# antekone/libarchive

Measured on AMD Instinct MI355X. Metric: decompressed MiB/s (whole node), lz4 filter, XXH32 verified, bit-exact, higher is better.
Workload: dtype u8; 1 GPU; C2: raw-format + lz4 filter, 16.00 GiB decoded per GPU, 262144 independent 64 KiB blocks per GPU in frames of 16, block+content+header XXH32 verified; compressed_bytes_per_gpu=7527480016, decoded_bytes_per_gpu=17179869184, unique_region_mib=1024, tiles=16, collectives=RCCL (nccl backend), expand_kernel=auto

## Files before the change

### include/la_gpu.h

```cpp
#ifndef LA_GPU_H
#define LA_GPU_H

#include <stddef.h>
#include <stdint.h>

#ifdef __cplusplus
extern "C" {
#endif

#define LA_GPU_ABI_VERSION 3

typedef enum la_rc {
	LA_OK            = 0,
	LA_ERR_NO_DEVICE = -1,
	LA_ERR_HIP       = -2,
	LA_ERR_ARG       = -3,
	LA_ERR_NOMEM     = -4
} la_rc;

typedef struct la_gpu_ctx la_gpu_ctx;

int         la_gpu_abi_version(void);
int         la_gpu_device_count(void);
int         la_gpu_open(int device, la_gpu_ctx **out);
// ... 116 lines not shown
	uint32_t flags;
	uint32_t content_sum;
	uint32_t reserved;
} la_lz4_frame;

typedef struct la_batch_summary {
	uint64_t total_out;
	uint32_t n_bad_units;
	uint32_t n_bad_frames;
	uint32_t first_bad_unit;
	uint32_t first_bad_frame;
	uint32_t first_zero_unit;
	uint32_t reserved;
} la_batch_summary;

#define LA_LZ4_OPT_GENERAL_ONLY 1u
#define LA_LZ4_OPT_NO_VERIFY    2u
#define LA_LZ4_OPT_PARSE_V1     4u

#define LA_LZ4_OPT_EXPAND_INORDER 8u

#define LA_LZ4_OPT_SEARCH_IN_EXPAND 16u

typedef struct la_lz4_batch {
	const uint8_t      *d_src;
	uint64_t            src_bytes;
	const la_lz4_block *d_blocks;
	uint32_t            n_blocks;
	const la_lz4_frame *d_frames;
	uint32_t            n_frames;
	uint8_t            *d_dst;
	uint64_t            dst_cap;
	uint32_t           *d_out_len;
	uint64_t           *d_dst_off;
	uint32_t           *d_block_status;
	uint32_t           *d_frame_status;
	la_batch_summary   *d_summary;
	uint32_t            options;
	uint32_t            hist_len;
	const void         *d_carry_in;
	void               *d_carry_out;
} la_lz4_batch;
#define LA_XXH_CARRY_BYTES 64u

uint64_t la_gpu_lz4_workspace_bytes(uint32_t n_blocks, uint64_t src_bytes);

// ... 453 lines not shown
```

### libarchive_amd/_native.py

```python
import ctypes as C
import os

import numpy as np

_PKG = os.path.dirname(os.path.abspath(__file__))
GPU_LIB_PATH = os.environ.get("LA_GPU_LIB") or os.path.join(_PKG, "csrc", "libla_gpu.so")
HOST_LIB_PATH = os.path.join(_PKG, "host", "libla_host.so")

LA_OK = 0

LZ4_BLOCK_DTYPE = np.dtype([("src_off", "<u8"), ("src_len", "<u4"), ("dst_cap", "<u4"),
                            ("flags", "<u4"), ("block_sum", "<u4")])
LZ4_FRAME_DTYPE = np.dtype([("desc_off", "<u8"), ("desc_len", "<u4"), ("first_block", "<u4"),
                            ("n_blocks", "<u4"), ("flags", "<u4"), ("content_sum", "<u4"),
                            ("reserved", "<u4")])
HASH_JOB_DTYPE = np.dtype([("off", "<u8"), ("len", "<u4"), ("seed", "<u4")])
SUMMARY_DTYPE = np.dtype([("total_out", "<u8"), ("n_bad_units", "<u4"), ("n_bad_frames", "<u4"),
                          ("first_bad_unit", "<u4"), ("first_bad_frame", "<u4"),
                          ("first_zero_unit", "<u4"), ("reserved", "<u4")])
GZ_MEMBER_DTYPE = np.dtype([("src_off", "<u8"), ("src_len", "<u4"), ("dst_cap", "<u4"), ("dst_off", "<u8")])
GZ_RESULT_DTYPE = np.dtype([("status", "<u4"), ("out_len", "<u4"), ("consumed", "<u4"), ("crc32", "<u4")])
assert LZ4_BLOCK_DTYPE.itemsize == 24 and LZ4_FRAME_DTYPE.itemsize == 32
assert HASH_JOB_DTYPE.itemsize == 16 and SUMMARY_DTYPE.itemsize == 32

LA_LZ4B_STORED, LA_LZ4B_CHECKSUM, LA_LZ4B_DEPENDENT, LA_LZ4B_FIRST = 1, 2, 4, 8
LA_LZ4F_CONTENT_SUM, LA_LZ4F_HEADER_SUM, LA_LZ4F_CONT, LA_LZ4F_OPEN, LA_LZ4F_HASHED = 1, 2, 4, 8, 16
LA_LZ4_OPT_GENERAL_ONLY, LA_LZ4_OPT_NO_VERIFY, LA_LZ4_OPT_PARSE_V1, LA_LZ4_OPT_EXPAND_INORDER = 1, 2, 4, 8
LA_LZ4_OPT_SEARCH_IN_EXPAND = 16
LA_GPU_ABI_VERSION = 3
LA_ST_OK, LA_ST_GZ_DATA, LA_ST_GZ_TRUNCATED, LA_ST_GZ_OUT_FULL, LA_ST_GZ_NO_TRAILER = 0, 5, 6, 9, 10
LA_ST_GZ_PIECE_END, LA_ST_GZ_NEEDS_HISTORY = 18, 19
(LA_GZ_OPT_NO_VERIFY, LA_GZ_OPT_WAVE_KERNEL, LA_GZ_OPT_LANE_KERNEL, LA_GZ_OPT_TWO_PHASE, LA_GZ_OPT_RAW,
 LA_GZ_OPT_EXPAND_INORDER, LA_GZ_OPT_PIECES) = 1, 2, 4, 8, 16, 32, 64
LA_GZ_OPT_CHAIN = 128
LA_GZ_OPT_BLOCK_STARTS = 256
LA_GZ_OPT_START_BIT_SHIFT = 16

(LA_END_EOF, LA_END_TRUNCATED, LA_END_MALFORMED, LA_END_MALFORMED_SKIP, LA_END_EMPTY_FRAME,
 LA_END_NEED_MORE, LA_END_GZ_NO_TRAILER, LA_END_GZ_TOO_LARGE) = range(8)


class NativeLibraryMissing(RuntimeError):
    pass


class _Lz4BatchC(C.Structure):
    _fields_ = [
        ("d_src", C.c_void_p), ("src_bytes", C.c_uint64),
        ("d_blocks", C.c_void_p), ("n_blocks", C.c_uint32),
        ("d_frames", C.c_void_p), ("n_frames", C.c_uint32),
        ("d_dst", C.c_void_p), ("dst_cap", C.c_uint64),
# ... 558 lines not shown
```

### libarchive_amd/csrc/la_api.hip

```cpp
#include "la_dev.h"
#include <stdio.h>
#include <stdlib.h>
#include <string.h>
#include <new>

#define LA_MAX_SLICES 8
#define LA_GZ_LANES_MIN 8192u
#define LA_PROF_MAX_RANGES 64

struct la_gpu_ctx {
	int device;
	hipStream_t own_stream;
	hipStream_t stream;
	hipEvent_t ev0, ev1;
	hipEvent_t mark;
	void *ws;
	uint64_t ws_bytes;
	uint32_t *lz4_deps;
	uint64_t lz4_deps_cap;
	uint8_t *lz4_plan;
	hipStream_t aux_stream;
	hipEvent_t slice_ev[LA_MAX_SLICES + 1];
	int prof_on;
	int prof_n;
	hipEvent_t prof_a[LA_PROF_MAX_RANGES], prof_b[LA_PROF_MAX_RANGES];
	const char *prof_name[LA_PROF_MAX_RANGES];
	char err[256];
};

static void prof_begin(la_gpu_ctx *c) { c->prof_n = 0; }
static int prof_open(la_gpu_ctx *c, const char *name, hipStream_t s)
{
	if (!c->prof_on || c->prof_n >= LA_PROF_MAX_RANGES)
		return -1;
	int h = c->prof_n++;
	c->prof_name[h] = name;
	(void)hipEventRecord(c->prof_a[h], s);
	return h;
}
static void prof_close(la_gpu_ctx *c, int h, hipStream_t s)
{
	if (h >= 0)
		(void)hipEventRecord(c->prof_b[h], s);
}

// ... 34 lines not shown
	*out = NULL;
	int n = 0;
	if (hipGetDeviceCount(&n) != hipSuccess || n <= 0 || device < 0 || device >= n)
		return LA_ERR_NO_DEVICE;
	la_gpu_ctx *c = new (std::nothrow) la_gpu_ctx();
	if (!c)
		return LA_ERR_NOMEM;
	memset(c, 0, sizeof(*c));
	c->device = device;
	if (hipSetDevice(device) != hipSuccess ||
	    hipStreamCreateWithFlags(&c->own_stream, hipStreamNonBlocking) != hipSuccess ||
	    hipEventCreate(&c->ev0) != hipSuccess || hipEventCreate(&c->ev1) != hipSuccess ||
	    hipEventCreateWithFlags(&c->mark, hipEventDisableTiming) != hipSuccess) {
		delete c;
		return LA_ERR_NO_DEVICE;
	}
	for (int i = 0; i < LA_PROF_MAX_RANGES; i++) {
		(void)hipEventCreate(&c->prof_a[i]);
		(void)hipEventCreate(&c->prof_b[i]);
	}
	(void)hipStreamCreateWithFlags(&c->aux_stream, hipStreamNonBlocking);
	for (int i = 0; i <= LA_MAX_SLICES; i++)
		(void)hipEventCreateWithFlags(&c->slice_ev[i], hipEventDisableTiming);
	c->stream = c->own_stream;
	*out = c;
	return LA_OK;
}

void la_gpu_close(la_gpu_ctx *c)
{
	if (!c)
		return;
	(void)hipSetDevice(c->device);
	(void)hipStreamSynchronize(c->stream);
	if (c->ws) (void)hipFree(c->ws);
	if (c->lz4_deps) (void)hipFree(c->lz4_deps);
	if (c->lz4_plan) (void)hipFree(c->lz4_plan);
	(void)hipEventDestroy(c->ev0);
	(void)hipEventDestroy(c->ev1);
	(void)hipEventDestroy(c->mark);
	for (int i = 0; i < LA_PROF_MAX_RANGES; i++) {
		(void)hipEventDestroy(c->prof_a[i]);
		(void)hipEventDestroy(c->prof_b[i]);
	}
	for (int i = 0; i <= LA_MAX_SLICES; i++)
		(void)hipEventDestroy(c->slice_ev[i]);
	(void)hipStreamSynchronize(c->aux_stream);
	(void)hipStreamDestroy(c->aux_stream);
	(void)hipStreamDestroy(c->own_stream);
	delete c;
}

int la_gpu_set_stream(la_gpu_ctx *c, void *hip_stream)
{
	if (!c) return LA_ERR_ARG;
	c->stream = hip_stream ? (hipStream_t)hip_stream : c->own_stream;
	return LA_OK;
}

int la_gpu_sync(la_gpu_ctx *c)
{
	if (!c) return LA_ERR_ARG;
	HIPCHK(c, hipStreamSynchronize(c->stream));
	return LA_OK;
}

const char *la_gpu_last_error(const la_gpu_ctx *c) { return c ? c->err : "no context"; }

int la_gpu_reserve(la_gpu_ctx *c, uint64_t bytes)
// ... 179 lines not shown
{
	lz4_ws w;
	lz4_ws_carve(&w, NULL, n_blocks, src_bytes, true);
	return w.total;
}

static int lz4_deps_reserve(la_gpu_ctx *c, uint64_t words)
{
	if (words <= c->lz4_deps_cap)
		return LA_OK;
	HIPCHK(c, hipSetDevice(c->device));
	HIPCHK(c, hipStreamSynchronize(c->stream));
	HIPCHK(c, hipStreamSynchronize(c->aux_stream));
	c->lz4_deps_cap = 0;
	if (c->lz4_deps) { HIPCHK(c, hipFree(c->lz4_deps)); c->lz4_deps = NULL; }
	if (c->lz4_plan) { HIPCHK(c, hipFree(c->lz4_plan)); c->lz4_plan = NULL; }
	words = (words + 0x3FFFFull) & ~0x3FFFFull;
	HIPCHK(c, hipMalloc((void **)&c->lz4_deps, words * sizeof(uint32_t)));
	HIPCHK(c, hipMalloc((void **)&c->lz4_plan, words));
	c->lz4_deps_cap = words;
	return LA_OK;
}

static bool lz4_uses_deps(const la_lz4_batch *bt)
{
	return !(bt->options & (LA_LZ4_OPT_GENERAL_ONLY | LA_LZ4_OPT_SEARCH_IN_EXPAND)) && bt->n_blocks &&
	    ((bt->options & LA_LZ4_OPT_EXPAND_INORDER) == 0 || !la_lz4_expand_inorder_takes(bt->src_bytes));
}

int la_gpu_lz4_decode(la_gpu_ctx *c, const la_lz4_batch *bt)
{
	if (!c || !bt)
		return LA_ERR_ARG;
	if (!bt->d_dst_off || (bt->n_blocks && (!bt->d_src || !bt->d_blocks || !bt->d_dst || !bt->d_out_len ||
	    !bt->d_block_status)))
		return LA_ERR_ARG;
	if (bt->n_frames && (!bt->d_frames || !bt->d_frame_status))
		return LA_ERR_ARG;
	const bool fast = !(bt->options & LA_LZ4_OPT_GENERAL_ONLY);
	const bool verify = !(bt->options & LA_LZ4_OPT_NO_VERIFY);
	const bool poll = (bt->options & LA_LZ4_OPT_EXPAND_INORDER) == 0 || !la_lz4_expand_inorder_takes(bt->src_bytes);
	lz4_ws w;
	lz4_ws_carve(&w, NULL, bt->n_blocks, bt->src_bytes, fast);
	if (w.total > c->ws_bytes) {
		int rc = la_gpu_reserve(c, w.total);
		if (rc != LA_OK) return rc;
	}
	lz4_ws_carve(&w, (uint8_t *)c->ws, bt->n_blocks, bt->src_bytes, fast);
	const bool with_deps = lz4_uses_deps(bt);
	if (with_deps) {
		int rc = lz4_deps_reserve(c, w.table_cap);
		if (rc != LA_OK) return rc;
	}
	hipStream_t sx = c->stream;
	hipStream_t sp = c->aux_stream;
	const uint32_t n = bt->n_blocks;
	const la_expand_job xj = {	 bt->d_src, bt->src_bytes, bt->d_blocks, n, bt->d_dst, bt->dst_cap, bt->d_dst_off,
	    bt->d_out_len, bt->d_block_status, w.nseq, fast ? w.table : NULL, w.table_off,
	    LA_LZ4_LONG_SEQ_BYTES,
	    with_deps ? c->lz4_deps : NULL, with_deps ? c->lz4_plan : NULL };

	prof_begin(c);
	HIPCHK(c, hipEventRecord(c->slice_ev[LA_MAX_SLICES], sx));
	HIPCHK(c, hipStreamWaitEvent(sp, c->slice_ev[LA_MAX_SLICES], 0));

	if (n)
		HIPCHK(c, hipMemsetAsync(bt->d_block_status, 0, (size_t)n * sizeof(uint32_t), sp));
	if (fast) {
		la_launch_lz4_table_caps(sp, bt->d_blocks, n, w.caps);
		la_launch_scan_u32(sp, w.caps, n, w.table_off, w.scan);
	}
	if (verify && n)
		HIPCHK(c, hipMemsetAsync(w.sum_status, 0, (size_t)n * sizeof(uint32_t), sp));
	if (bt->options & LA_LZ4_OPT_PARSE_V1) {
		if (verify && n)
			prof_range(c, "lz4_block_sums", sp, [&] { la_launch_lz4_block_sums(sp, bt->d_src, bt->d_blocks, n, w.sum_status); });
		prof_range(c, "lz4_parse", sp, [&] {
			la_launch_lz4_parse(sp, bt->d_src, bt->src_bytes, bt->d_blocks, n, bt->d_out_len, w.nseq,
			    bt->d_block_status, fast ? w.table : NULL, w.table_off, w.table_cap);
		});
	} else {
		prof_range(c, "lz4_parse", sp, [&] {
			la_launch_lz4_parse_staged(sp, bt->d_src, bt->src_bytes, bt->d_blocks, n, bt->d_out_len, w.nseq,
			    bt->d_block_status, verify ? w.sum_status : NULL, fast ? w.table : NULL, w.table_off, w.table_cap);
		});
	}
	HIPCHK(c, hipEventRecord(c->slice_ev[0], sp));

	HIPCHK(c, hipStreamWaitEvent(sx, c->slice_ev[0], 0));
	prof_range(c, "scan", sx, [&] { la_launch_scan_u32(sx, bt->d_out_len, n, bt->d_dst_off, w.scan); });
	if (with_deps)
		prof_range(c, "lz4_deps", sx, [&] { la_launch_lz4_deps(sx, xj, c->lz4_deps, c->lz4_plan); });

	prof_range(c, fast ? "lz4_expand_general" : "lz4_expand", sx, [&] { la_launch_lz4_expand_general(sx, xj, bt->hist_len); });
	if (fast && poll)
		prof_range(c, "lz4_expand_big", sx, [&] { la_launch_lz4_expand_fast_big(sx, xj, w.big); });
	const uint32_t nsl = (fast && n >= 4u * 8192u) ? 4u : 1u;
	if (bt->n_frames && !verify)
		HIPCHK(c, hipMemsetAsync(bt->d_frame_status, 0, (size_t)bt->n_frames * sizeof(uint32_t), sx));
	for (uint32_t i = 0; i < nsl; i++) {
		const uint32_t first = (uint32_t)((uint64_t)n * i / nsl), last = (uint32_t)((uint64_t)n * (i + 1) / nsl);
		const la_expand_job sj = xj.slice(first, last - first);
		if (fast)
			prof_range(c, "lz4_expand", sx, [&] { (poll ? la_launch_lz4_expand_fast : la_launch_lz4_expand_inorder)(sx, sj); });
		if (bt->n_frames && verify) {
			HIPCHK(c, hipEventRecord(c->slice_ev[1 + i], sx));
			HIPCHK(c, hipStreamWaitEvent(sp, c->slice_ev[1 + i], 0));
			prof_range(c, "lz4_frame_sums", sp, [&] {
				la_launch_lz4_frame_sums(sp, bt->d_src, bt->d_dst, bt->d_frames, bt->n_frames,
				    bt->d_dst_off, bt->dst_cap, bt->d_frame_status, i ? first + 1 : 0u, last,
				    bt->d_carry_in, bt->d_carry_out,
				    i + 1 == nsl);
			});
		}
	}
	HIPCHK(c, hipEventRecord(c->slice_ev[LA_MAX_SLICES - 1], sp));
	HIPCHK(c, hipStreamWaitEvent(sx, c->slice_ev[LA_MAX_SLICES - 1], 0));
	if (verify)
		la_launch_lz4_merge_status(sx, w.sum_status, n, bt->d_block_status);
	if (bt->d_summary)
		prof_range(c, "summary", sx, [&] {
			la_launch_lz4_summary(sx, bt->d_out_len, bt->d_block_status, n, bt->d_frame_status, bt->n_frames, bt->d_dst_off, bt->d_summary);
		});
	HIPCHK(c, hipGetLastError());
// ... 671 lines not shown
```

### libarchive_amd/csrc/la_dev.h

```cpp
#ifndef LA_DEV_H
#define LA_DEV_H

#include <hip/hip_runtime.h>
#include <stdint.h>
#include "../../include/la_gpu.h"

#define LA_WAVE 64

__device__ __forceinline__ uint32_t ld_u32(const uint8_t *p)
{
	uint32_t v;
	__builtin_memcpy(&v, p, 4);
	return v;
}
__device__ __forceinline__ uint4 ld_u128(const uint8_t *p)
{
	uint4 v;
	__builtin_memcpy(&v, p, 16);
	return v;
}
__device__ __forceinline__ uint32_t rotl32(uint32_t x, int r)
{
	return __builtin_rotateleft32(x, r);
}

#define XXH_P1 0x9E3779B1u
#define XXH_P2 0x85EBCA77u
#define XXH_P3 0xC2B2AE3Du
// ... 332 lines not shown
	uint64_t off;
	template <typename T> T *take(uint64_t count, uint64_t align = alignof(T))
	{
		off = (off + align - 1) & ~(align - 1);
		T *p = base ? (T *)(void *)(base + off) : nullptr;
		off += count * sizeof(T);
		return p;
	}
};


void la_launch_xxh32_many(hipStream_t s, const uint8_t *d_base, const la_hash_job *d_jobs,
    uint32_t n, uint32_t *d_out);
void la_launch_crc32_many(hipStream_t s, const uint8_t *d_base, const la_hash_job *d_jobs,
    uint32_t n, uint32_t *d_out);
void la_launch_adler32_many(hipStream_t s, const uint8_t *d_base, const la_hash_job *d_jobs,
    uint32_t n, uint32_t *d_out);
void la_launch_lz4_block_sums(hipStream_t s, const uint8_t *d_src, const la_lz4_block *d_blocks,
    uint32_t n, uint32_t *d_status);
void la_launch_lz4_frame_sums(hipStream_t s, const uint8_t *d_src, const uint8_t *d_dst,
    const la_lz4_frame *d_frames, uint32_t n_frames, const uint64_t *d_dst_off,
    uint64_t dst_cap, uint32_t *d_frame_status, uint32_t end_lo, uint32_t end_hi,
    const void *d_carry_in, void *d_carry_out, int row );
void la_launch_lz4_merge_status(hipStream_t s, const uint32_t *d_sum_status, uint32_t n, uint32_t *d_status);

struct la_lz4_seq {
	uint16_t lit_src;
	uint16_t lit_len;
	uint16_t dst;
	uint16_t off;
};

#define LA_LZ4_FAST_MAXSEQ 4096u
#define LA_INFLATE_MAXSEQ 12288u

__host__ __device__ __forceinline__ bool la_lz4_fast_eligible(const la_lz4_block &b)
{
	return !(b.flags & (LA_LZ4B_STORED | LA_LZ4B_DEPENDENT)) && b.dst_cap <= 65536u && b.src_len <= 65536u;
}

#define LA_LZ4_LONG_SEQ_BYTES 512u
__host__ __device__ __forceinline__ bool la_lz4_long_sequences(uint32_t nseq, uint32_t out_len, uint32_t thr)
{
	return thr != 0 && nseq != 0xFFFFFFFFu && (uint64_t)nseq * thr <= out_len;
}

// ... 125 lines not shown
	uint32_t long_thr;
	const uint32_t *deps;
	const uint8_t *lit_plan;

	la_expand_job slice(uint32_t first, uint32_t count) const
	{
		return la_expand_job{ src, src_bytes, blocks + first, count, dst, dst_cap, dst_off + first, out_len + first,
		    status + first, nseq + first, table, table_off + first, long_thr, deps, lit_plan };
	}
};

void la_launch_lz4_table_caps(hipStream_t s, const la_lz4_block *d_blocks, uint32_t n, uint32_t *d_caps);
void la_launch_lz4_parse(hipStream_t s, const uint8_t *d_src, uint64_t src_bytes,
    const la_lz4_block *d_blocks, uint32_t n, uint32_t *d_out_len, uint32_t *d_nseq,
    uint32_t *d_status, la_lz4_seq *d_table , const uint64_t *d_table_off,
    uint64_t table_cap );
void la_launch_lz4_parse_staged(hipStream_t s, const uint8_t *d_src, uint64_t src_bytes,
    const la_lz4_block *d_blocks, uint32_t n, uint32_t *d_out_len, uint32_t *d_nseq,
    uint32_t *d_status, uint32_t *d_sum_status, la_lz4_seq *d_table, const uint64_t *d_table_off,
    uint64_t table_cap);
void la_launch_lz4_expand_general(hipStream_t s, const la_expand_job &j, uint32_t hist_len);
void la_launch_lz4_expand_fast(hipStream_t s, const la_expand_job &j);
void la_launch_lz4_expand_fast_big(hipStream_t s, const la_expand_job &j, uint32_t *d_big );
void la_launch_lz4_deps(hipStream_t s, const la_expand_job &j, uint32_t *d_deps, uint8_t *d_plan);

bool la_lz4_expand_inorder_takes(uint64_t src_bytes);
void la_launch_lz4_expand_inorder(hipStream_t s, const la_expand_job &j);

uint64_t la_zstd_workspace_bytes(uint32_t n_frames);
void la_launch_zstd_frames(hipStream_t s, const uint8_t *d_src, uint64_t src_bytes, const la_zstd_frame *d_frames, uint32_t n,
    uint8_t *d_dst, uint64_t dst_cap, la_zstd_result *d_results, uint8_t *ws, uint32_t options,
    const uint32_t *d_only );
uint64_t la_zstd_blocks_workspace_bytes(uint32_t n_frames, uint64_t src_bytes, uint64_t dst_cap);
const uint32_t *la_zstd_blocks_todo(const uint8_t *ws);
void la_launch_zstd_blocks(hipStream_t s, const uint8_t *d_src, uint64_t src_bytes, const la_zstd_frame *d_frames, uint32_t n,
    uint8_t *d_dst, uint64_t dst_cap, la_zstd_result *d_results, uint8_t *ws, uint32_t options);

uint64_t la_bzip2_workspace_bytes(uint32_t n, uint32_t level);
uint32_t la_bzip2_max_blocks(uint32_t level);
uint64_t la_bzip2_scan_ws_bytes(uint64_t src_bytes);
void la_launch_bzip2_scan(hipStream_t s, const uint8_t *d_src, uint64_t src_bytes, la_bz2_cand *d_cands, uint32_t cap,
    uint32_t *d_count, uint8_t *ws);
void la_launch_bzip2_measure(hipStream_t s, const la_bz2_batch *bt, uint8_t *ws);
void la_launch_bzip2_walk(hipStream_t s, const la_bz2_batch *bt, uint8_t *ws);
void la_launch_bzip2_emit(hipStream_t s, const la_bz2_batch *bt, uint8_t *ws);
void la_launch_bzip2_verify(hipStream_t s, const la_bz2_batch *bt, uint8_t *ws);
// ... 134 lines not shown
```

### libarchive_amd/csrc/la_hash.hip

```cpp
#include "la_dev.h"


__global__ __launch_bounds__(256) void xxh32_many_kernel(const uint8_t *__restrict__ base,
    const la_hash_job *__restrict__ jobs, uint32_t n, uint32_t *__restrict__ out)
{
	uint32_t i = blockIdx.x * blockDim.x + threadIdx.x;
	if (i >= n)
		return;
	la_hash_job j = jobs[i];
	out[i] = xxh32_lane(base + j.off, j.len, j.seed);
}

__global__ __launch_bounds__(256) void lz4_merge_status_kernel(const uint32_t *__restrict__ sum_status,
    uint32_t n, uint32_t *__restrict__ status)
{
	uint32_t i = blockIdx.x * blockDim.x + threadIdx.x;
	if (i < n && sum_status[i] != LA_ST_OK)
		status[i] = sum_status[i];
}

void la_launch_lz4_merge_status(hipStream_t s, const uint32_t *d_sum_status, uint32_t n, uint32_t *d_status)
{
	if (n == 0) return;
	hipLaunchKernelGGL(lz4_merge_status_kernel, dim3((n + 255) / 256), dim3(256), 0, s, d_sum_status, n, d_status);
// ... 119 lines not shown
			cout->total_lo = (uint32_t)total;
			cout->total_hi = (uint32_t)(total >> 32);
			for (int k = 0; k < 16; k++) cout->mem[k] = mem[k];
		}
		return 0;
	}
	uint32_t h;
	const int rot = (j == 0) ? 1 : (j == 1) ? 7 : (j == 2) ? 12 : 18;
	uint32_t t = rotl32(v, rot);
	t += __shfl_xor(t, 1, 64);
	t += __shfl_xor(t, 2, 64);
	h = total >= 16 ? t : XXH_P5;
	h += (uint32_t)total;
	uint32_t k = 0;
	for (; k + 4 <= msz; k += 4) {
		const uint32_t dw = (uint32_t)mem[k] | ((uint32_t)mem[k + 1] << 8) | ((uint32_t)mem[k + 2] << 16) | ((uint32_t)mem[k + 3] << 24);
		h = rotl32(h + dw * XXH_P3, 17) * XXH_P4;
	}
	for (; k < msz; k++)
		h = rotl32(h + (uint32_t)mem[k] * XXH_P5, 11) * XXH_P1;
	return xxh_avalanche(h);
}

template <bool ROW>
__global__ __launch_bounds__(64) void lz4_frame_sums_kernel(const uint8_t *__restrict__ src,
    const uint8_t *__restrict__ dst, const la_lz4_frame *__restrict__ frames, uint32_t n,
    const uint64_t *__restrict__ dst_off, uint64_t dst_cap, uint32_t *__restrict__ fstatus,
    uint32_t end_lo, uint32_t end_hi, const la_xxh_carry *carry_in, la_xxh_carry *carry_out)
{
	uint32_t t = blockIdx.x * blockDim.x + threadIdx.x;
	uint32_t i = ROW ? t >> 4 : t >> 2;
	const int l = (int)(t & (ROW ? 15u : 3u));
	int j = l & 3;
	if (i >= n)
		return;
	la_lz4_frame f = frames[i];
	const uint32_t fend = f.first_block + f.n_blocks;
	if (fend < end_lo || fend > end_hi)
		return;
	uint32_t st = LA_ST_OK;
	if (f.flags & LA_LZ4F_HEADER_SUM) {
		uint32_t h = xxh32_quad(src + f.desc_off, f.desc_len - 1, 0, j);
		if (((h >> 8) & 0xff) != src[f.desc_off + f.desc_len - 1])
			st = LA_ST_LZ4_BAD_HEADER_SUM;
	}
	if (st == LA_ST_OK && (f.flags & (LA_LZ4F_CONT | LA_LZ4F_OPEN))) {
		if ((f.flags & LA_LZ4F_HASHED) && carry_in && carry_out) {
			uint64_t a = dst_off[f.first_block], e = dst_off[f.first_block + f.n_blocks];
			if (e <= dst_cap) {
				const uint32_t h = xxh32_quad_stream<ROW>((f.flags & LA_LZ4F_CONT) ? carry_in : nullptr,
				    (f.flags & LA_LZ4F_OPEN) ? carry_out : nullptr, dst + a, e - a, l);
				if (!(f.flags & LA_LZ4F_OPEN) && (f.flags & LA_LZ4F_CONTENT_SUM) && h != f.content_sum)
					st = LA_ST_LZ4_BAD_CONTENT_SUM;
			}
		}
	} else if (st == LA_ST_OK && (f.flags & LA_LZ4F_CONTENT_SUM)) {
		uint64_t a = dst_off[f.first_block], e = dst_off[f.first_block + f.n_blocks];
		if (e <= dst_cap) {
			uint32_t h = ROW ? xxh32_row(dst + a, (uint32_t)(e - a), 0, l) : xxh32_quad(dst + a, (uint32_t)(e - a), 0, j);
			if (h != f.content_sum)
				st = LA_ST_LZ4_BAD_CONTENT_SUM;
		}
	}
	if (l == 0)
		fstatus[i] = st;
}

void la_launch_xxh32_many(hipStream_t s, const uint8_t *d_base, const la_hash_job *d_jobs,
    uint32_t n, uint32_t *d_out)
{
	if (n == 0) return;
	hipLaunchKernelGGL(xxh32_many_kernel, dim3((n + 255) / 256), dim3(256), 0, s, d_base, d_jobs, n, d_out);
}

void la_launch_lz4_block_sums(hipStream_t s, const uint8_t *d_src, const la_lz4_block *d_blocks,
    uint32_t n, uint32_t *d_status)
{
	if (n == 0) return;
	hipLaunchKernelGGL(lz4_block_sums_kernel, dim3((n + 255) / 256), dim3(256), 0, s, d_src, d_blocks, n, d_status);
}

void la_launch_lz4_frame_sums(hipStream_t s, const uint8_t *d_src, const uint8_t *d_dst,
    const la_lz4_frame *d_frames, uint32_t n_frames, const uint64_t *d_dst_off, uint64_t dst_cap,
    uint32_t *d_frame_status, uint32_t end_lo, uint32_t end_hi, const void *d_carry_in, void *d_carry_out,
    int row)
{
	if (n_frames == 0) return;
	if (row)
		hipLaunchKernelGGL(lz4_frame_sums_kernel<true>, dim3((n_frames + 3) / 4), dim3(64), 0, s,
		    d_src, d_dst, d_frames, n_frames, d_dst_off, dst_cap, d_frame_status, end_lo, end_hi,
		    (const la_xxh_carry *)d_carry_in, (la_xxh_carry *)d_carry_out);
	else
		hipLaunchKernelGGL(lz4_frame_sums_kernel<false>, dim3((n_frames + 15) / 16), dim3(64), 0, s,
		    d_src, d_dst, d_frames, n_frames, d_dst_off, dst_cap, d_frame_status, end_lo, end_hi,
		    (const la_xxh_carry *)d_carry_in, (la_xxh_carry *)d_carry_out);
}


#define CRC_POLY 0xEDB88320u

__device__ __forceinline__ uint32_t gf2_mulmod(uint32_t a, uint32_t b)
{
	uint32_t r = 0;
#pragma unroll 8
	for (int i = 0; i < 32; i++) {
		r ^= b & (0u - (a >> 31));
		a <<= 1;
		b = (b >> 1) ^ (CRC_POLY & (0u - (b & 1)));
	}
	return r;
}

__device__ uint32_t gf2_xpow8(uint32_t nbytes)
{
	uint32_t result = 0x80000000u, base = 0x00800000u;
	while (nbytes) {
		if (nbytes & 1)
			result = gf2_mulmod(result, base);
// ... 388 lines not shown
```

### libarchive_amd/csrc/la_lz4_fast.hip

```cpp
#include "la_dev.h"

#ifndef POLL_SLEEP
#define POLL_SLEEP 1
#endif
#ifndef FAST_THREADS
#define FAST_THREADS 512
#endif
#ifndef LBATCH
#define LBATCH 2
#endif
#ifndef FAST_MIN_WAVES
#define FAST_MIN_WAVES 4
#endif
#define FAST_WAVES   (FAST_THREADS / 64)

#ifdef LA_DIAG
__device__ unsigned long long *la_diag_stamps;
#define STAMP(slot)                                                                       \
	do {                                                                              \
		if (threadIdx.x == 0 && la_diag_stamps)                                    \
			la_diag_stamps[(size_t)blockIdx.x * 8 + (slot)] = __builtin_readcyclecounter(); \
	} while (0)
#else
#define STAMP(slot) do { } while (0)
#endif

typedef uint64_t seq_t;

#ifndef STEP_SHIFT
#define STEP_SHIFT  2u
#endif
#define STEP_SEQS   (1u << STEP_SHIFT)
#define STEP_LANES  (64u >> STEP_SHIFT)
#define STEPS_PER_SLOT (64u >> STEP_SHIFT)
__device__ __forceinline__ uint32_t fast_seq_index(uint32_t r, uint32_t wave, uint32_t lane)
{
	return (((r * STEPS_PER_SLOT + (lane >> STEP_SHIFT)) * FAST_WAVES + wave) << STEP_SHIFT) + (lane & (STEP_SEQS - 1));
}
__device__ __forceinline__ seq_t seq_load(const la_lz4_seq *t, uint32_t k)
{
	return *(const uint64_t *)(const void *)(t + k);
}
#define SEQ_LIT_SRC(e) ((uint32_t)((e) & 0xFFFFu))
#define SEQ_LIT_LEN(e) ((uint32_t)(((e) >> 16) & 0xFFFFu))
#define SEQ_DST(e)     ((uint32_t)(((e) >> 32) & 0xFFFFu))
#define SEQ_OFF(e)     ((uint32_t)((e) >> 48))

template <uint32_t MAXSEQ, bool SEG, bool DEPS>
__global__ __launch_bounds__(FAST_THREADS, FAST_MIN_WAVES) void lz4_expand_fast_kernel(
    const uint8_t *__restrict__ src, uint64_t src_bytes, const la_lz4_block *__restrict__ blocks,
    uint32_t n, uint8_t *__restrict__ dst, uint64_t dst_cap, const uint64_t *__restrict__ dst_off,
    const uint32_t *__restrict__ out_len, uint32_t *status_out,
    const uint32_t *__restrict__ nseq, const la_lz4_seq *__restrict__ table,
    const uint64_t *__restrict__ table_off, const uint32_t *__restrict__ big_list,
    const uint32_t *__restrict__ big_count, uint32_t long_thr, const uint32_t *__restrict__ deps,
    const uint8_t *__restrict__ lit_plan)
{
	static_assert(!(SEG && DEPS), "the dependency words number a block's sequences from its first one");
	const uint32_t *status = status_out;
	__shared__ __attribute__((aligned(16))) uint8_t win[16 + 65536 + 96];
	__shared__ uint16_t dstpos[MAXSEQ + 4];
	__shared__ uint32_t donebits[MAXSEQ / 32];
	__shared__ uint16_t chunk_first[DEPS ? 8 : 2048 + 8];

	auto do_block = [&](const uint32_t bi) __attribute__((always_inline)) {
	if (bi >= n)
		return;
	const la_lz4_block_words b = la_lz4_load_block_words<true, SEG>(bi, blocks, status, out_len, nseq, dst_off, table_off);
	LA_PIN_SCALARS("s"(src), "s"(src_bytes), "s"(dst), "s"(dst_cap), "s"(table), "s"(long_thr), "s"(deps), "s"(lit_plan));
	const uint32_t olen = b.out_len;
	const uint32_t ns_all = b.nseq;
	const uint64_t doff = b.dst_off;
	static_assert(MAXSEQ == LA_LZ4_FAST_MAXSEQ, "la_lz4_route splits the window kernels' blocks at LA_LZ4_FAST_MAXSEQ");
	if (la_lz4_route_words(b, dst_cap, true, long_thr) != (SEG ? LA_XR_WINDOW_SEG : LA_XR_WINDOW))
		return;

	STAMP(0);
	const uint32_t tid = threadIdx.x, lane = tid & 63, wave = tid >> 6;
	const la_lz4_seq *const tab_all = table + b.table_off;
	const uint8_t *s = src + b.src_off;
	const uint64_t s_room = src_bytes - b.src_off;
// ... 462 lines not shown
	};
	if (!SEG) {
		segment(0u);
	} else {
		for (uint32_t kb = 0; kb < ns_all; kb += MAXSEQ)
			segment(kb);
	}
	STAMP(4);

	uint32_t head = (16u - (uint32_t)((uintptr_t)g_out & 15)) & 15u;
	if (head > olen) head = olen;
	if (tid < head)
		g_out[tid] = W[tid];
	const uint32_t nflush = (olen - head) >> 4;
	const uint4 *wsrc = (const uint4 *)(W + head);
	uint4 *gdst = (uint4 *)(g_out + head);
	for (uint32_t c = tid; c < nflush; c += FAST_THREADS)
		gdst[c] = wsrc[c];
	const uint32_t tail0 = head + (nflush << 4);
	if (tail0 + tid < olen)
		g_out[tail0 + tid] = W[tail0 + tid];
	STAMP(5);
	};
	if (!SEG) {
		do_block(blockIdx.x);
	} else {
		const uint32_t cnt = *big_count;
		for (uint32_t li = blockIdx.x; li < cnt; li += gridDim.x) {
			do_block(big_list[li]);
			__syncthreads();
		}
	}
}

__global__ __launch_bounds__(256) void lz4_classify_kernel(const la_lz4_block *__restrict__ blocks, uint32_t n,
    const uint32_t *__restrict__ status, const uint32_t *__restrict__ nseq, uint32_t *__restrict__ big_list,
    uint32_t *__restrict__ big_count, const uint32_t *__restrict__ out_len, uint32_t long_thr)
{
	const uint32_t i = blockIdx.x * blockDim.x + threadIdx.x;
	if (i >= n)
		return;
	if (la_lz4_route(blocks[i], status[i], out_len[i], nseq[i], 0, ~0ull, true, long_thr) == LA_XR_WINDOW_SEG)
		big_list[atomicAdd(big_count, 1u)] = i;
}

#ifdef LA_DIAG
extern "C" int la_diag_set_stamps(void *d_buf)
{
	unsigned long long *p = (unsigned long long *)d_buf;
	return (int)hipMemcpyToSymbol(HIP_SYMBOL(la_diag_stamps), &p, sizeof(p));
}
#endif

void la_launch_lz4_expand_fast(hipStream_t s, const la_expand_job &j)
{
	if (j.n == 0) return;
	if (j.deps && j.lit_plan)
		hipLaunchKernelGGL((lz4_expand_fast_kernel<LA_LZ4_FAST_MAXSEQ, false, true>), dim3(j.n), dim3(FAST_THREADS), 0, s,
		    j.src, j.src_bytes, j.blocks, j.n, j.dst, j.dst_cap, j.dst_off, j.out_len, j.status, j.nseq,
		    j.table, j.table_off, (const uint32_t *)nullptr, (const uint32_t *)nullptr, j.long_thr, j.deps, j.lit_plan);
	else
		hipLaunchKernelGGL((lz4_expand_fast_kernel<LA_LZ4_FAST_MAXSEQ, false, false>), dim3(j.n), dim3(FAST_THREADS), 0, s,
		    j.src, j.src_bytes, j.blocks, j.n, j.dst, j.dst_cap, j.dst_off, j.out_len, j.status, j.nseq,
		    j.table, j.table_off, (const uint32_t *)nullptr, (const uint32_t *)nullptr, j.long_thr, (const uint32_t *)nullptr,
		    (const uint8_t *)nullptr);
}

void la_launch_lz4_expand_fast_big(hipStream_t s, const la_expand_job &j, uint32_t *d_big)
{
	if (j.n == 0) return;
	(void)hipMemsetAsync(d_big, 0, sizeof(uint32_t), s);
	hipLaunchKernelGGL(lz4_classify_kernel, dim3((j.n + 255) / 256), dim3(256), 0, s, j.blocks, j.n, j.status, j.nseq,
	    d_big + 1, d_big, j.out_len, j.long_thr);
	const uint32_t grid = j.n < 1024u ? j.n : 1024u;
	hipLaunchKernelGGL((lz4_expand_fast_kernel<LA_LZ4_FAST_MAXSEQ, true, false>), dim3(grid), dim3(FAST_THREADS), 0, s,
	    j.src, j.src_bytes, j.blocks, j.n, j.dst, j.dst_cap, j.dst_off, j.out_len, j.status, j.nseq,
	    j.table, j.table_off, (const uint32_t *)(d_big + 1), (const uint32_t *)d_big, j.long_thr, (const uint32_t *)nullptr,
	    (const uint8_t *)nullptr);
}
```

Baseline: 695,100 MiB/s.

## Split last LZ4 expand slice into strided block groups overlapped with streamed frame hashing

The last expand slice is split into several groups that cover a range of block positions within each frame (periodic layout, 16 blocks per frame). After each group finishes, the frame XXH32 content-sum kernel on the aux stream hashes the now-ready prefix of every frame and stores a streaming carry. The final pass then only hashes the remaining part and checks the sum. The goal is to hide the verification tail that used to run after the last expand slice. In exchange it adds extra kernel launches, a carry buffer and event syncs, and the strided grids may launch with lower occupancy.

```diff
diff --git a/include/la_gpu.h b/include/la_gpu.h
--- a/include/la_gpu.h
+++ b/include/la_gpu.h
@@ -162,6 +162,8 @@
 
 #define LA_LZ4_OPT_SEARCH_IN_EXPAND 16u
 
+#define LA_LZ4_OPT_SPLIT_SMALL 32u
+
 typedef struct la_lz4_batch {
 	const uint8_t      *d_src;
 	uint64_t            src_bytes;
diff --git a/libarchive_amd/_native.py b/libarchive_amd/_native.py
--- a/libarchive_amd/_native.py
+++ b/libarchive_amd/_native.py
@@ -27,6 +27,7 @@
 LA_LZ4F_CONTENT_SUM, LA_LZ4F_HEADER_SUM, LA_LZ4F_CONT, LA_LZ4F_OPEN, LA_LZ4F_HASHED = 1, 2, 4, 8, 16
 LA_LZ4_OPT_GENERAL_ONLY, LA_LZ4_OPT_NO_VERIFY, LA_LZ4_OPT_PARSE_V1, LA_LZ4_OPT_EXPAND_INORDER = 1, 2, 4, 8
 LA_LZ4_OPT_SEARCH_IN_EXPAND = 16
+LA_LZ4_OPT_SPLIT_SMALL = 32
 LA_GPU_ABI_VERSION = 3
 LA_ST_OK, LA_ST_GZ_DATA, LA_ST_GZ_TRUNCATED, LA_ST_GZ_OUT_FULL, LA_ST_GZ_NO_TRAILER = 0, 5, 6, 9, 10
 LA_ST_GZ_PIECE_END, LA_ST_GZ_NEEDS_HISTORY = 18, 19
diff --git a/libarchive_amd/csrc/la_api.hip b/libarchive_amd/csrc/la_api.hip
--- a/libarchive_amd/csrc/la_api.hip
+++ b/libarchive_amd/csrc/la_api.hip
@@ -21,6 +21,9 @@
 	uint8_t *lz4_plan;
 	hipStream_t aux_stream;
 	hipEvent_t slice_ev[LA_MAX_SLICES + 1];
+	hipEvent_t split_ev[LA_LZ4_SPLIT_MAX_GROUPS];
+	void *lz4_carry;
+	uint64_t lz4_carry_cap;
 	int prof_on;
 	int prof_n;
 	hipEvent_t prof_a[LA_PROF_MAX_RANGES], prof_b[LA_PROF_MAX_RANGES];
@@ -101,6 +104,8 @@
 	(void)hipStreamCreateWithFlags(&c->aux_stream, hipStreamNonBlocking);
 	for (int i = 0; i <= LA_MAX_SLICES; i++)
 		(void)hipEventCreateWithFlags(&c->slice_ev[i], hipEventDisableTiming);
+	for (uint32_t i = 0; i < LA_LZ4_SPLIT_MAX_GROUPS; i++)
+		(void)hipEventCreateWithFlags(&c->split_ev[i], hipEventDisableTiming);
 	c->stream = c->own_stream;
 	*out = c;
 	return LA_OK;
@@ -115,6 +120,7 @@
 	if (c->ws) (void)hipFree(c->ws);
 	if (c->lz4_deps) (void)hipFree(c->lz4_deps);
 	if (c->lz4_plan) (void)hipFree(c->lz4_plan);
+	if (c->lz4_carry) (void)hipFree(c->lz4_carry);
 	(void)hipEventDestroy(c->ev0);
 	(void)hipEventDestroy(c->ev1);
 	(void)hipEventDestroy(c->mark);
@@ -124,6 +130,8 @@
 	}
 	for (int i = 0; i <= LA_MAX_SLICES; i++)
 		(void)hipEventDestroy(c->slice_ev[i]);
+	for (uint32_t i = 0; i < LA_LZ4_SPLIT_MAX_GROUPS; i++)
+		(void)hipEventDestroy(c->split_ev[i]);
 	(void)hipStreamSynchronize(c->aux_stream);
 	(void)hipStreamDestroy(c->aux_stream);
 	(void)hipStreamDestroy(c->own_stream);
@@ -349,6 +357,25 @@
 	return LA_OK;
 }
 
+static int lz4_carry_reserve(la_gpu_ctx *c, uint64_t records)
+{
+	if (records <= c->lz4_carry_cap)
+		return LA_OK;
+	HIPCHK(c, hipSetDevice(c->device));
+	HIPCHK(c, hipStreamSynchronize(c->stream));
+	HIPCHK(c, hipStreamSynchronize(c->aux_stream));
+	c->lz4_carry_cap = 0;
+	if (c->lz4_carry) { HIPCHK(c, hipFree(c->lz4_carry)); c->lz4_carry = NULL; }
+	records = (records + 0xFFFull) & ~0xFFFull;
+	HIPCHK(c, hipMalloc(&c->lz4_carry, records * LA_XXH_CARRY_BYTES));
+	c->lz4_carry_cap = records;
+	return LA_OK;
+}
+
+static const uint32_t lz4_split_sixteenths[] = { 8, 13, 16 };
+static_assert(sizeof(lz4_split_sixteenths) / sizeof(lz4_split_sixteenths[0]) <= LA_LZ4_SPLIT_MAX_GROUPS, "too many groups");
+static const bool lz4_split_row_hidden = false;
+
 static bool lz4_uses_deps(const la_lz4_batch *bt)
 {
 	return !(bt->options & (LA_LZ4_OPT_GENERAL_ONLY | LA_LZ4_OPT_SEARCH_IN_EXPAND)) && bt->n_blocks &&
@@ -379,9 +406,21 @@
 		int rc = lz4_deps_reserve(c, w.table_cap);
 		if (rc != LA_OK) return rc;
 	}
+	const uint32_t n = bt->n_blocks;
+	const uint32_t nsl = (fast && n >= 4u * 8192u) ? 4u : 1u;
+	la_lz4_split split = { 0, 0, 0, 0, { 0 } };
+	if (fast && poll && with_deps && verify && bt->n_frames && (nsl == 4 || (bt->options & LA_LZ4_OPT_SPLIT_SMALL))) {
+		const uint32_t P = la_lz4_split_period(n, bt->n_frames);
+		if (P) {
+			const uint32_t first = nsl == 4 ? (uint32_t)((uint64_t)n * 3 / 4) / P * P : 0u;
+			la_lz4_split_init(&split, first, n, P, lz4_split_sixteenths,
+			    sizeof(lz4_split_sixteenths) / sizeof(lz4_split_sixteenths[0]));
+			int rc = lz4_carry_reserve(c, n - first);
+			if (rc != LA_OK) return rc;
+		}
+	}
 	hipStream_t sx = c->stream;
 	hipStream_t sp = c->aux_stream;
-	const uint32_t n = bt->n_blocks;
 	const la_expand_job xj = {	 bt->d_src, bt->src_bytes, bt->d_blocks, n, bt->d_dst, bt->dst_cap, bt->d_dst_off,
 	    bt->d_out_len, bt->d_block_status, w.nseq, fast ? w.table : NULL, w.table_off,
 	    LA_LZ4_LONG_SEQ_BYTES,
@@ -422,11 +461,28 @@
 	prof_range(c, fast ? "lz4_expand_general" : "lz4_expand", sx, [&] { la_launch_lz4_expand_general(sx, xj, bt->hist_len); });
 	if (fast && poll)
 		prof_range(c, "lz4_expand_big", sx, [&] { la_launch_lz4_expand_fast_big(sx, xj, w.big); });
-	const uint32_t nsl = (fast && n >= 4u * 8192u) ? 4u : 1u;
 	if (bt->n_frames && !verify)
 		HIPCHK(c, hipMemsetAsync(bt->d_frame_status, 0, (size_t)bt->n_frames * sizeof(uint32_t), sx));
 	for (uint32_t i = 0; i < nsl; i++) {
-		const uint32_t first = (uint32_t)((uint64_t)n * i / nsl), last = (uint32_t)((uint64_t)n * (i + 1) / nsl);
+		uint32_t first = (uint32_t)((uint64_t)n * i / nsl), last = (uint32_t)((uint64_t)n * (i + 1) / nsl);
+		if (split.n_groups) {
+			if (i + 2 == nsl)
+				last = split.first;
+			if (i + 1 == nsl) {
+				for (uint32_t g = 0; g < split.n_groups; g++) {
+					prof_range(c, "lz4_expand", sx, [&] { la_launch_lz4_expand_fast_group(sx, xj, split, g); });
+					HIPCHK(c, hipEventRecord(c->split_ev[g], sx));
+					HIPCHK(c, hipStreamWaitEvent(sp, c->split_ev[g], 0));
+					const bool tail = g + 1 == split.n_groups;
+					prof_range(c, tail ? "lz4_frame_sums_tail" : "lz4_frame_sums", sp, [&] {
+						la_launch_lz4_frame_sums_split(sp, bt->d_src, bt->d_dst, bt->d_frames, bt->n_frames,
+						    bt->d_dst_off, bt->dst_cap, bt->d_frame_status, split, g, c->lz4_carry,
+						    bt->d_carry_in, bt->d_carry_out, tail || lz4_split_row_hidden);
+					});
+				}
+				break;
+			}
+		}
 		const la_expand_job sj = xj.slice(first, last - first);
 		if (fast)
 			prof_range(c, "lz4_expand", sx, [&] { (poll ? la_launch_lz4_expand_fast : la_launch_lz4_expand_inorder)(sx, sj); });
diff --git a/libarchive_amd/csrc/la_dev.h b/libarchive_amd/csrc/la_dev.h
--- a/libarchive_amd/csrc/la_dev.h
+++ b/libarchive_amd/csrc/la_dev.h
@@ -4,6 +4,7 @@
 #include <hip/hip_runtime.h>
 #include <stdint.h>
 #include "../../include/la_gpu.h"
+#include "la_lz4_slices.h"
 
 #define LA_WAVE 64
 
@@ -382,6 +383,10 @@
     const la_lz4_frame *d_frames, uint32_t n_frames, const uint64_t *d_dst_off,
     uint64_t dst_cap, uint32_t *d_frame_status, uint32_t end_lo, uint32_t end_hi,
     const void *d_carry_in, void *d_carry_out, int row );
+void la_launch_lz4_frame_sums_split(hipStream_t s, const uint8_t *d_src, const uint8_t *d_dst,
+    const la_lz4_frame *d_frames, uint32_t n_frames, const uint64_t *d_dst_off, uint64_t dst_cap,
+    uint32_t *d_frame_status, const la_lz4_split &sp, uint32_t g, void *d_carries, const void *d_carry_in,
+    void *d_carry_out, int row);
 void la_launch_lz4_merge_status(hipStream_t s, const uint32_t *d_sum_status, uint32_t n, uint32_t *d_status);
 
 struct la_lz4_seq {
@@ -553,6 +558,7 @@
 void la_launch_lz4_expand_general(hipStream_t s, const la_expand_job &j, uint32_t hist_len);
 void la_launch_lz4_expand_fast(hipStream_t s, const la_expand_job &j);
 void la_launch_lz4_expand_fast_big(hipStream_t s, const la_expand_job &j, uint32_t *d_big );
+void la_launch_lz4_expand_fast_group(hipStream_t s, const la_expand_job &j, const la_lz4_split &sp, uint32_t g);
 void la_launch_lz4_deps(hipStream_t s, const la_expand_job &j, uint32_t *d_deps, uint8_t *d_plan);
 
 bool la_lz4_expand_inorder_takes(uint64_t src_bytes);
diff --git a/libarchive_amd/csrc/la_hash.hip b/libarchive_amd/csrc/la_hash.hip
--- a/libarchive_amd/csrc/la_hash.hip
+++ b/libarchive_amd/csrc/la_hash.hip
@@ -165,11 +165,20 @@
 	return xxh_avalanche(h);
 }
 
-template <bool ROW>
+template <bool SPLIT> struct frame_sums_pass { };
+template <> struct frame_sums_pass<true> {
+	uint32_t first, period;
+	uint32_t h_lo, h_hi;
+	uint32_t last_pass;
+	la_xxh_carry *carries;
+};
+
+template <bool ROW, bool SPLIT = false>
 __global__ __launch_bounds__(64) void lz4_frame_sums_kernel(const uint8_t *__restrict__ src,
     const uint8_t *__restrict__ dst, const la_lz4_frame *__restrict__ frames, uint32_t n,
     const uint64_t *__restrict__ dst_off, uint64_t dst_cap, uint32_t *__restrict__ fstatus,
-    uint32_t end_lo, uint32_t end_hi, const la_xxh_carry *carry_in, la_xxh_carry *carry_out)
+    uint32_t end_lo, uint32_t end_hi, const la_xxh_carry *carry_in, la_xxh_carry *carry_out,
+    const frame_sums_pass<SPLIT> pass)
 {
 	uint32_t t = blockIdx.x * blockDim.x + threadIdx.x;
 	uint32_t i = ROW ? t >> 4 : t >> 2;
@@ -181,13 +190,40 @@
 	const uint32_t fend = f.first_block + f.n_blocks;
 	if (fend < end_lo || fend > end_hi)
 		return;
+	bool streamed = false;
+	uint32_t lo = 0, hi = 0;
+	la_xxh_carry *carry = nullptr;
+	if constexpr (SPLIT) {
+		if (f.n_blocks && (f.flags & (LA_LZ4F_CONTENT_SUM | LA_LZ4F_CONT | LA_LZ4F_OPEN)) == LA_LZ4F_CONTENT_SUM) {
+			const uint64_t a = dst_off[f.first_block], e = dst_off[fend];
+			streamed = e <= dst_cap && e - a <= 0xFFFFFFFFull;
+		}
+		if (streamed) {
+			lo = la_lz4_split_pass_lo(pass.first, pass.period, pass.h_lo, f.first_block, f.n_blocks);
+			hi = la_lz4_split_ready(pass.first, pass.period, pass.h_hi, f.first_block, f.n_blocks);
+			carry = pass.carries + la_lz4_split_carry_index(pass.first, f.first_block, f.n_blocks);
+		}
+		if (!pass.last_pass) {
+			if (hi > lo) {
+				const uint64_t a = dst_off[f.first_block + lo], e = dst_off[f.first_block + hi];
+				(void)xxh32_quad_stream<ROW>(lo ? carry : nullptr, carry, dst + a, e - a, l);
+			}
+			return;
+		}
+	}
 	uint32_t st = LA_ST_OK;
 	if (f.flags & LA_LZ4F_HEADER_SUM) {
 		uint32_t h = xxh32_quad(src + f.desc_off, f.desc_len - 1, 0, j);
 		if (((h >> 8) & 0xff) != src[f.desc_off + f.desc_len - 1])
 			st = LA_ST_LZ4_BAD_HEADER_SUM;
 	}
-	if (st == LA_ST_OK && (f.flags & (LA_LZ4F_CONT | LA_LZ4F_OPEN))) {
+	if (SPLIT && streamed) {
+		if (st == LA_ST_OK) {
+			const uint64_t a = dst_off[f.first_block + lo], e = dst_off[f.first_block + hi];
+			if (xxh32_quad_stream<ROW>(lo ? carry : nullptr, nullptr, dst + a, e - a, l) != f.content_sum)
+				st = LA_ST_LZ4_BAD_CONTENT_SUM;
+		}
+	} else if (st == LA_ST_OK && (f.flags & (LA_LZ4F_CONT | LA_LZ4F_OPEN))) {
 		if ((f.flags & LA_LZ4F_HASHED) && carry_in && carry_out) {
 			uint64_t a = dst_off[f.first_block], e = dst_off[f.first_block + f.n_blocks];
 			if (e <= dst_cap) {
@@ -230,13 +266,32 @@
 {
 	if (n_frames == 0) return;
 	if (row)
-		hipLaunchKernelGGL(lz4_frame_sums_kernel<true>, dim3((n_frames + 3) / 4), dim3(64), 0, s,
+		hipLaunchKernelGGL((lz4_frame_sums_kernel<true, false>), dim3((n_frames + 3) / 4), dim3(64), 0, s,
 		    d_src, d_dst, d_frames, n_frames, d_dst_off, dst_cap, d_frame_status, end_lo, end_hi,
-		    (const la_xxh_carry *)d_carry_in, (la_xxh_carry *)d_carry_out);
+		    (const la_xxh_carry *)d_carry_in, (la_xxh_carry *)d_carry_out, frame_sums_pass<false>{});
 	else
-		hipLaunchKernelGGL(lz4_frame_sums_kernel<false>, dim3((n_frames + 15) / 16), dim3(64), 0, s,
+		hipLaunchKernelGGL((lz4_frame_sums_kernel<false, false>), dim3((n_frames + 15) / 16), dim3(64), 0, s,
 		    d_src, d_dst, d_frames, n_frames, d_dst_off, dst_cap, d_frame_status, end_lo, end_hi,
-		    (const la_xxh_carry *)d_carry_in, (la_xxh_carry *)d_carry_out);
+		    (const la_xxh_carry *)d_carry_in, (la_xxh_carry *)d_carry_out, frame_sums_pass<false>{});
+}
+
+void la_launch_lz4_frame_sums_split(hipStream_t s, const uint8_t *d_src, const uint8_t *d_dst,
+    const la_lz4_frame *d_frames, uint32_t n_frames, const uint64_t *d_dst_off, uint64_t dst_cap,
+    uint32_t *d_frame_status, const la_lz4_split &sp, uint32_t g, void *d_carries, const void *d_carry_in,
+    void *d_carry_out, int row)
+{
+	if (n_frames == 0) return;
+	const frame_sums_pass<true> pass = { sp.first, sp.period, sp.bound[g], sp.bound[g + 1], g + 1 == sp.n_groups,
+	    (la_xxh_carry *)d_carries };
+	const uint32_t end_lo = sp.first ? sp.first + 1 : 0u;
+	if (row)
+		hipLaunchKernelGGL((lz4_frame_sums_kernel<true, true>), dim3((n_frames + 3) / 4), dim3(64), 0, s,
+		    d_src, d_dst, d_frames, n_frames, d_dst_off, dst_cap, d_frame_status, end_lo, sp.last,
+		    (const la_xxh_carry *)d_carry_in, (la_xxh_carry *)d_carry_out, pass);
+	else
+		hipLaunchKernelGGL((lz4_frame_sums_kernel<false, true>), dim3((n_frames + 15) / 16), dim3(64), 0, s,
+		    d_src, d_dst, d_frames, n_frames, d_dst_off, dst_cap, d_frame_status, end_lo, sp.last,
+		    (const la_xxh_carry *)d_carry_in, (la_xxh_carry *)d_carry_out, pass);
 }
 
 
diff --git a/libarchive_amd/csrc/la_lz4_fast.hip b/libarchive_amd/csrc/la_lz4_fast.hip
--- a/libarchive_amd/csrc/la_lz4_fast.hip
+++ b/libarchive_amd/csrc/la_lz4_fast.hip
@@ -46,17 +46,23 @@
 #define SEQ_DST(e)     ((uint32_t)(((e) >> 32) & 0xFFFFu))
 #define SEQ_OFF(e)     ((uint32_t)((e) >> 48))
 
-template <uint32_t MAXSEQ, bool SEG, bool DEPS>
+struct fast_stride { uint32_t base, period; };
+template <bool STRIDED> struct fast_list_arg { typedef const uint32_t *__restrict__ type; };
+template <> struct fast_list_arg<true> { typedef fast_stride type; };
+static_assert(sizeof(fast_stride) == sizeof(const uint32_t *), "the stride takes the list's place");
+
+template <uint32_t MAXSEQ, bool SEG, bool DEPS, bool STRIDED = false>
 __global__ __launch_bounds__(FAST_THREADS, FAST_MIN_WAVES) void lz4_expand_fast_kernel(
     const uint8_t *__restrict__ src, uint64_t src_bytes, const la_lz4_block *__restrict__ blocks,
     uint32_t n, uint8_t *__restrict__ dst, uint64_t dst_cap, const uint64_t *__restrict__ dst_off,
     const uint32_t *__restrict__ out_len, uint32_t *status_out,
     const uint32_t *__restrict__ nseq, const la_lz4_seq *__restrict__ table,
-    const uint64_t *__restrict__ table_off, const uint32_t *__restrict__ big_list,
+    const uint64_t *__restrict__ table_off, typename fast_list_arg<STRIDED>::type big_list ,
     const uint32_t *__restrict__ big_count, uint32_t long_thr, const uint32_t *__restrict__ deps,
     const uint8_t *__restrict__ lit_plan)
 {
 	static_assert(!(SEG && DEPS), "the dependency words number a block's sequences from its first one");
+	static_assert(!(SEG && STRIDED), "the segmented launch takes its blocks from a list");
 	const uint32_t *status = status_out;
 	__shared__ __attribute__((aligned(16))) uint8_t win[16 + 65536 + 96];
 	__shared__ uint16_t dstpos[MAXSEQ + 4];
@@ -565,7 +571,9 @@
 		g_out[tail0 + tid] = W[tail0 + tid];
 	STAMP(5);
 	};
-	if (!SEG) {
+	if constexpr (STRIDED) {
+		do_block(la_lz4_split_block(big_list.base, big_list.period, blockIdx.x, blockIdx.y));
+	} else if constexpr (!SEG) {
 		do_block(blockIdx.x);
 	} else {
 		const uint32_t cnt = *big_count;
@@ -609,6 +617,16 @@
 		    (const uint8_t *)nullptr);
 }
 
+void la_launch_lz4_expand_fast_group(hipStream_t s, const la_expand_job &j, const la_lz4_split &sp, uint32_t g)
+{
+	const uint32_t gx = la_lz4_split_grid_x(&sp, g), gy = la_lz4_split_grid_y(&sp, g);
+	if (gx == 0 || gy == 0) return;
+	const fast_stride st = { sp.first + sp.bound[g], sp.period };
+	hipLaunchKernelGGL((lz4_expand_fast_kernel<LA_LZ4_FAST_MAXSEQ, false, true, true>), dim3(gx, gy), dim3(FAST_THREADS), 0, s,
+	    j.src, j.src_bytes, j.blocks, sp.last, j.dst, j.dst_cap, j.dst_off, j.out_len, j.status, j.nseq,
+	    j.table, j.table_off, st, (const uint32_t *)nullptr, j.long_thr, j.deps, j.lit_plan);
+}
+
 void la_launch_lz4_expand_fast_big(hipStream_t s, const la_expand_job &j, uint32_t *d_big)
 {
 	if (j.n == 0) return;
diff --git a/libarchive_amd/csrc/la_lz4_slices.h b/libarchive_amd/csrc/la_lz4_slices.h
--- /dev/null
+++ b/libarchive_amd/csrc/la_lz4_slices.h
@@ -0,0 +1,88 @@
+#ifndef LA_LZ4_SLICES_H
+#define LA_LZ4_SLICES_H
+
+#include <stdint.h>
+
+#if defined(__HIPCC__)
+#define LA_SLICE_FN __host__ __device__ static inline
+#else
+#define LA_SLICE_FN static inline
+#endif
+
+#define LA_LZ4_SPLIT_MAX_GROUPS 4u
+#define LA_LZ4_SPLIT_MIN_PERIOD 4u
+#define LA_LZ4_SPLIT_MAX_PERIOD 64u
+
+typedef struct la_lz4_split {
+	uint32_t first, last;
+	uint32_t period;
+	uint32_t n_groups;
+	uint32_t bound[LA_LZ4_SPLIT_MAX_GROUPS + 1];
+} la_lz4_split;
+
+LA_SLICE_FN uint32_t la_lz4_split_period(uint32_t n_blocks, uint32_t n_frames)
+{
+	if (n_frames == 0 || n_blocks % n_frames != 0)
+		return 0;
+	const uint32_t p = n_blocks / n_frames;
+	return (p >= LA_LZ4_SPLIT_MIN_PERIOD && p <= LA_LZ4_SPLIT_MAX_PERIOD) ? p : 0;
+}
+
+LA_SLICE_FN void la_lz4_split_init(la_lz4_split *sp, uint32_t first, uint32_t last, uint32_t period,
+    const uint32_t *sixteenths, uint32_t n)
+{
+	sp->first = first;
+	sp->last = last;
+	sp->period = period;
+	sp->bound[0] = 0;
+	uint32_t g = 0;
+	for (uint32_t k = 0; k < n; k++) {
+		const uint32_t h = k + 1 == n ? period : period * sixteenths[k] / 16u;
+		if (h > sp->bound[g] && h <= period)
+			sp->bound[++g] = h;
+	}
+	sp->n_groups = g;
+}
+
+LA_SLICE_FN uint32_t la_lz4_split_group_blocks(const la_lz4_split *sp, uint32_t g)
+{
+	const uint32_t len = sp->last - sp->first, whole = len / sp->period, rest = len % sp->period;
+	const uint32_t lo = sp->bound[g], hi = sp->bound[g + 1];
+	return whole * (hi - lo) + (rest > lo ? (rest < hi ? rest : hi) - lo : 0u);
+}
+
+LA_SLICE_FN uint32_t la_lz4_split_grid_x(const la_lz4_split *sp, uint32_t g)
+{
+	const uint32_t len = sp->last - sp->first, lo = sp->bound[g];
+	return len > lo ? (len - lo + sp->period - 1u) / sp->period : 0u;
+}
+LA_SLICE_FN uint32_t la_lz4_split_grid_y(const la_lz4_split *sp, uint32_t g)
+{
+	return sp->bound[g + 1] - sp->bound[g];
+}
+LA_SLICE_FN uint32_t la_lz4_split_block(uint32_t base, uint32_t period, uint32_t x, uint32_t y)
+{
+	return base + x * period + y;
+}
+
+LA_SLICE_FN uint32_t la_lz4_split_ready(uint32_t first, uint32_t period, uint32_t h, uint32_t first_block, uint32_t n_blocks)
+{
+	if (h >= period)
+		return n_blocks;
+	const uint32_t s = first_block > first ? first_block : first;
+	const uint32_t r = (s - first) % period;
+	const uint32_t stop = r < h ? s + (h - r) : s;
+	const uint32_t run = stop - first_block;
+	return run < n_blocks ? run : n_blocks;
+}
+
+LA_SLICE_FN uint32_t la_lz4_split_pass_lo(uint32_t first, uint32_t period, uint32_t h_lo, uint32_t first_block, uint32_t n_blocks)
+{
+	return h_lo == 0 ? 0u : la_lz4_split_ready(first, period, h_lo, first_block, n_blocks);
+}
+LA_SLICE_FN uint32_t la_lz4_split_carry_index(uint32_t first, uint32_t first_block, uint32_t n_blocks)
+{
+	return first_block + n_blocks - 1u - first;
+}
+
+#endif
```

Measured after the change: 705,300 MiB/s (median of 6 runs). +1.5%, better.
